# pycompression/python-zlib-ng

Measured on AMD Instinct MI355X. Metric: MB/s compress+decompress, 128 KiB blocks level 6, higher is better.
Workload: dtype u8

## Files before the change

### python-zlib-ng_amd/build.py

```python
import os
import subprocess
import sys

HERE = os.path.dirname(os.path.abspath(__file__))
CSRC = os.path.join(HERE, "csrc")
OUT = os.path.join(HERE, "zlib_ng_amd", "libzng_amd.so")
SOURCES = ["zng_amd.hip"]
DEPS = ["zng_amd.hip", "zng_stream.hip", "za_common.h", "za_crc.h", "za_deflate.hip", "za_inflate.hip", "za_inflate_units.hip", "za_inflate_spans.hip", "za_batch.hip", "za_dict.hip", "za_checksum.hip",
        os.path.join("..", "..", "include", "zng_amd.h")]


def needs_build():
    if not os.path.exists(OUT):
        return True
    t = os.path.getmtime(OUT)
    return any(os.path.getmtime(os.path.join(CSRC, d)) > t for d in DEPS)


def build(force=False, verbose=False):
    if not force and not needs_build():
        return OUT
    hipcc = os.environ.get("HIPCC", "/opt/rocm/bin/hipcc")
    cmd = [hipcc, "--offload-arch=gfx950", "-O3", "-std=c++17", "-fPIC", "-shared",
           "-Wall", "-Wno-unused-variable", "-Wno-unused-but-set-variable",
           "-o", OUT] + [os.path.join(CSRC, s) for s in SOURCES]
    if verbose:
        print(" ".join(cmd))
    subprocess.check_call(cmd)
    return OUT


def build_host_asan(out):
    hipcc = os.environ.get("HIPCC", "/opt/rocm/bin/hipcc")
    cmd = [hipcc, "--offload-arch=gfx950", "-Wno-option-ignored", "-O1", "-g", "-std=c++17", "-fPIC", "-shared", "-fsanitize=address,undefined",
           "-fno-sanitize-recover=undefined", "-fno-omit-frame-pointer", "-o", out] + [os.path.join(CSRC, s) for s in SOURCES]
    subprocess.check_call(cmd)
    return out


if __name__ == "__main__":
    if "--host-asan" in sys.argv:
        print(build_host_asan(sys.argv[sys.argv.index("--host-asan") + 1]))
    else:
        print(build(force="--force" in sys.argv, verbose=True))
```

### python-zlib-ng_amd/csrc/za_deflate.hip

```cpp
#include "za_common.h"
#include "za_crc.h"
#include <type_traits>

#define ZA_CH_GROUP 16
#define ZA_CH_OFFS(x) (((x) >> (32 - ZA_HASH_BITS - 2)) & (((1u << ZA_HASH_BITS) - 1u) << 2))
#define ZA_CH_CHUNK (64 * ZA_CH_GROUP)

typedef uint32_t za_v4u32 __attribute__((ext_vector_type(4)));
__device__ __forceinline__ void za_issue_load16(za_v4u32 &dst, const uint8_t *addr)
{
    asm volatile("global_load_dwordx4 %0, %1, off" : "=v"(dst) : "v"(addr) : "memory");
}
template <int NEWER>
__device__ __forceinline__ void za_wait_loads(za_v4u32 &a, za_v4u32 &b, za_v4u32 &c, za_v4u32 &d)
{
    asm volatile("s_waitcnt vmcnt(%4)" : "+v"(a), "+v"(b), "+v"(c), "+v"(d) : "n"(NEWER) : "memory");
}

__device__ __noinline__ uint32_t za_chains_fix(uint32_t h, uint32_t A, uint32_t old, bool ins)
{
    uint32_t near = 0, pre = 0xFFFFFFFFu;
    const int lane = za_lane();
    const unsigned long long insm = __ballot(ins);
    for (int j = 0; j < 64; j++) {
        const uint32_t hj = (uint32_t)__builtin_amdgcn_readlane((int)h, j), Aj = (uint32_t)__builtin_amdgcn_readlane((int)A, j);
        const uint32_t oj = (uint32_t)__builtin_amdgcn_readlane((int)old, j);
        if (((insm >> j) & 1ull) != 0ull && hj == h) {
            if (j < lane) near = Aj;
            pre = oj < pre ? oj : pre;
        }
    }
    return near ? near : pre;
}

#ifdef ZA_CH_STATS
__device__ unsigned long long za_ch_stat[32];
#endif
template <int TABLE>
__global__ __launch_bounds__(256) void za_k_chains(const uint8_t *__restrict__ in, const ZaUnit *__restrict__ units,
                                                   const uint32_t *__restrict__ run_start,
                                                   uint16_t *__restrict__ prev_ws,
                                                   uint32_t *__restrict__ cost_ws = nullptr)
{
    __shared__ uint32_t head[1 << ZA_HASH_BITS];
    __shared__ __attribute__((aligned(16))) uint32_t ring[(2 * ZA_CH_CHUNK + 16) / 4];
    __shared__ __attribute__((aligned(16))) uint16_t hbuf[2][ZA_CH_CHUNK];
    __shared__ __attribute__((aligned(16))) uint32_t obuf[2][ZA_CH_CHUNK];
    constexpr int HB = ZaTableBytes<TABLE>::value;
    const uint32_t lane = (uint32_t)za_lane();
    const uint32_t role = threadIdx.x >> 6;
    const uint32_t u0 = run_start[blockIdx.x], u1 = run_start[blockIdx.x + 1];
#ifdef ZA_CH_STATS
    unsigned long long st_wait = 0, st_ph[4] = {0, 0, 0, 0};
    const unsigned long long st_t0 = clock64();
#endif
    uint32_t goff = 0;
    uint32_t n_prev = 0;
#pragma unroll 1
    for (uint32_t ui = u0; ui < u1; ui++) {
        const ZaUnit u = units[ui];
        const int n = (int)u.in_len, dict_len = (int)u.dict_len;
        if (cost_ws && threadIdx.x == 0) cost_ws[(size_t)ui * ZA_DP_COSTS + 258] = 0u;
        const uint8_t *row = in + u.in_off - dict_len;
        uint16_t *prevdist = prev_ws + (size_t)ui * ZA_PREV_STRIDE;
#ifdef ZA_ABL_NO_CARRY
        const bool carry = false;
#else
        const bool carry = ui > u0 && (u.flags & ZA_FLAG_CARRY) != 0u;
#endif
        if (carry) goff += n_prev;
        else {
            goff = 0;
            for (uint32_t i = threadIdx.x * 4u; i < (1u << ZA_HASH_BITS); i += 1024u) *(uint4 *)&head[i] = make_uint4(0u, 0u, 0u, 0u);
        }
        __syncthreads();
        n_prev = (uint32_t)n;
        const int total = dict_len + n;
        const int first = carry ? dict_len - (HB - 1) : 0;
        const uint32_t abase = goff + (uint32_t)(2 * ZA_WIN - dict_len) + 1u;
        if (total < HB) {
            if (role == 2u && (int)lane >= first && (int)lane < total) prevdist[lane] = 0;
            continue;
        }
        if (total < 16) {
            if (role == 2u) {
                uint32_t h = 0xFFFFFFFFu;
                const bool ins = (int)lane >= first && (int)lane <= total - HB;
                if (ins) {
                    uint32_t w[3] = {0u, 0u, 0u};
#pragma unroll
                    for (int b = 0; b < HB; b++) w[b >> 2] |= (uint32_t)row[lane + b] << (8 * (b & 3));
                    h = za_hash_x<TABLE>(w[0], w[1], w[2]) >> (32 - ZA_HASH_BITS);
                }
                uint32_t d = 0;
                for (int j = 0; j < 16; j++) {
                    const uint32_t hj = (uint32_t)__builtin_amdgcn_readlane((int)h, j);
                    if (ins && j < (int)lane && hj == h) d = lane - (uint32_t)j;
                }
                if ((int)lane >= first && (int)lane < total) prevdist[lane] = (uint16_t)d;
            }
            continue;
        }
        const int iclamp_hi = total - HB;
        const int t0 = first & ~63;
        const int ngroups = (total - t0 + ZA_CH_CHUNK - 1) / ZA_CH_CHUNK;
        const int last16 = total - 16;
        auto fetch = [&](int c, za_v4u32 &dst) {
            int at = t0 + c * ZA_CH_CHUNK + 16 * (int)lane;
            at = at > last16 ? last16 : at;
            za_issue_load16(dst, row + at);
        };
        auto stage = [&](int c, uint4 v) {
            const int cbase = t0 + c * ZA_CH_CHUNK;
            if (cbase + ZA_CH_CHUNK > total) {
                const int at = cbase + 16 * (int)lane;
                const int delta = at > last16 ? at - last16 : 0;
                const uint32_t w[8] = {v.x, v.y, v.z, v.w, 0u, 0u, 0u, 0u};
                uint32_t r[4];
#pragma unroll
                for (int i = 0; i < 4; i++) {
                    uint32_t lo = 0, hi = 0;
#pragma unroll
                    for (int j = 0; j < 8; j++) { lo = (i + (delta >> 2)) == j ? w[j] : lo; hi = (i + (delta >> 2) + 1) == j ? w[j] : hi; }
                    r[i] = delta >= 16 ? 0u : __builtin_amdgcn_alignbyte(hi, lo, (uint32_t)delta & 3u);
                }
                v = make_uint4(r[0], r[1], r[2], r[3]);
            }
            *(uint4 *)(ring + (c & 1) * (ZA_CH_CHUNK / 4) + 4 * lane) = v;
            if ((c & 1) == 0 && lane == 0) *(uint4 *)(ring + 2 * ZA_CH_CHUNK / 4) = v;
        };
        auto hash_half = [&](int k, int g0, uint16_t *hb) {
#ifdef ZA_ABL_CH_NOHASH
            return;
#endif
            const uint32_t *w = ring + (k & 1) * (ZA_CH_CHUNK / 4) + 16 * g0 + lane;
            uint16_t *o = hb + 64 * g0 + 4 * lane;
#pragma unroll
            for (int j = 0; j < ZA_CH_GROUP / 8; j++) {
                const uint32_t d0 = w[64 * j], d1 = w[64 * j + 1];
                uint32_t hh[4];
                if constexpr (TABLE == ZA_TABLE_A) {
                    hh[0] = za_hash_x<TABLE>(d0, d1, 0u);
#pragma unroll
                    for (int q = 1; q < 4; q++) hh[q] = za_hash_x<TABLE>(__builtin_amdgcn_alignbyte(d1, d0, q), d1 >> (8 * q), 0u);
                } else if constexpr (TABLE == ZA_TABLE_B) {
                    hh[0] = za_hash_x<TABLE>(d0, 0u, 0u);
#pragma unroll
                    for (int q = 1; q < 4; q++) hh[q] = za_hash_x<TABLE>(__builtin_amdgcn_alignbyte(d1, d0, q), 0u, 0u);
                } else {
                    const uint32_t d2 = w[64 * j + 2], d3 = w[64 * j + 3];
                    hh[0] = za_hash_x<TABLE>(d0, d1, d2);
#pragma unroll
                    for (int q = 1; q < 4; q++)
                        hh[q] = za_hash_x<TABLE>(__builtin_amdgcn_alignbyte(d1, d0, q), __builtin_amdgcn_alignbyte(d2, d1, q), __builtin_amdgcn_alignbyte(d3, d2, q));
                }
                *(uint2 *)(o + 256 * j) = make_uint2(ZA_CH_OFFS(hh[0]) | (ZA_CH_OFFS(hh[1]) << 16), ZA_CH_OFFS(hh[2]) | (ZA_CH_OFFS(hh[3]) << 16));
            }
        };
        auto group_inner = [&](int k) -> bool {
            const int tbase = t0 + k * ZA_CH_CHUNK;
            return tbase >= first && tbase + ZA_CH_CHUNK - 1 <= iclamp_hi;
        };
        auto insert_as = [&](auto inner_tag, int tbase, const uint16_t *hb, uint32_t *ob) {
            constexpr bool inner = decltype(inner_tag)::value;
            const uint32_t li = (uint32_t)tbase + lane;
            uint32_t hh[ZA_CH_GROUP], old[ZA_CH_GROUP];
            const uint32_t A0 = abase + li;
#ifdef ZA_CH_STATS
            const unsigned long long T0 = clock64();
#endif
#ifdef ZA_ABL_CH_HALFREADS
#pragma unroll
            for (int g = 0; g < ZA_CH_GROUP; g += 2) { const uint32_t t = *(const uint32_t *)&hb[64 * g + 2 * (lane >> 1)]; hh[g] = t & 0xFFFCu; hh[g + 1] = (t >> 16) & 0xFFFCu; }
#else
#pragma unroll
            for (int g = 0; g < ZA_CH_GROUP; g++) hh[g] = hb[64 * g + lane];
#endif
#ifdef ZA_CH_STATS
            asm volatile("s_waitcnt lgkmcnt(0)" ::: "memory");
            const unsigned long long T1 = clock64();
#endif
#pragma unroll
            for (int g = 0; g < ZA_CH_GROUP; g++) {
                const int i = (int)li + 64 * g;
                const bool ins = inner || (i >= first && i <= iclamp_hi);
                old[g] = 0u;
#ifdef ZA_ABL_CH_NOATOMIC
                if (ins) old[g] = *(const uint32_t *)((const uint8_t *)head + hh[g]);
#else
                if (ins) old[g] = atomicMax((uint32_t *)((uint8_t *)head + hh[g]), A0 + 64u * (uint32_t)g);
#endif
            }
#ifdef ZA_CH_STATS
            asm volatile("s_waitcnt lgkmcnt(0)" ::: "memory");
            const unsigned long long T2 = clock64();
#endif
            uint32_t top = 0;
#pragma unroll
            for (int g = 0; g < ZA_CH_GROUP; g++) top |= (A0 + 64u * (uint32_t)g - old[g] - 1u);
#ifndef ZA_ABL_CH_NOCHECK
            if (__builtin_expect(__ballot((int)top < 0) != 0ull, 0)) {
#pragma unroll 1
                for (int g = 0; g < ZA_CH_GROUP; g++) {
                    const int i = (int)li + 64 * g;
                    const bool ins = inner || (i >= first && i <= iclamp_hi);
                    const uint32_t A = A0 + 64u * (uint32_t)g;
                    uint32_t hg = hh[0], og = old[0];
#pragma unroll
                    for (int q = 1; q < ZA_CH_GROUP; q++) { hg = g == q ? hh[q] : hg; og = g == q ? old[q] : og; }
                    const uint32_t ofix = za_chains_fix(hg >> 2, A, og, ins);
#pragma unroll
                    for (int q = 0; q < ZA_CH_GROUP; q++) old[q] = g == q ? ofix : old[q];
                }
            }
#endif
#ifdef ZA_ABL_CH_HALFWRITES
#pragma unroll
            for (int g = 0; g < ZA_CH_GROUP; g += 2) ob[64 * g + lane] = old[g] + old[g + 1];
#else
#pragma unroll
            for (int g = 0; g < ZA_CH_GROUP; g++) ob[64 * g + lane] = old[g];
#endif
#ifdef ZA_CH_STATS
            asm volatile("s_waitcnt lgkmcnt(0)" ::: "memory");
            st_ph[0] += T1 - T0; st_ph[1] += T2 - T1; st_ph[2] += clock64() - T2; st_ph[3] += 1;
#endif
        };
        auto store_links = [&](int k, uint32_t *ob) {
            const int tbase = t0 + k * ZA_CH_CHUNK;
            const uint32_t A0 = abase + (uint32_t)tbase + lane;
            uint32_t dd[ZA_CH_GROUP];
#pragma unroll
            for (int g = 0; g < ZA_CH_GROUP; g++) dd[g] = A0 + 64u * (uint32_t)g - ob[64 * g + lane];
            if (group_inner(k)) {
                uint16_t *lb = (uint16_t *)ob;
                __builtin_amdgcn_fence(__ATOMIC_ACQ_REL, "wavefront");
                __builtin_amdgcn_wave_barrier();
#pragma unroll
                for (int g = 0; g < ZA_CH_GROUP; g++) lb[64 * g + lane] = (uint16_t)(dd[g] <= (uint32_t)ZA_WIN ? dd[g] : 0u);
                __builtin_amdgcn_fence(__ATOMIC_ACQ_REL, "wavefront");
                __builtin_amdgcn_wave_barrier();
                const uint4 v0 = *(const uint4 *)&lb[8 * lane], v1 = *(const uint4 *)&lb[512 + 8 * lane];
#ifndef ZA_ABL_CH_NOSTORE
                *(uint4 *)(prevdist + tbase + 8 * (int)lane) = v0;
                *(uint4 *)(prevdist + tbase + 512 + 8 * (int)lane) = v1;
#endif
            } else {
#pragma unroll
                for (int g = 0; g < ZA_CH_GROUP; g++) {
                    const int i = tbase + (int)lane + 64 * g;
                    if (i >= first && i < total) prevdist[i] = (uint16_t)((i <= iclamp_hi && dd[g] <= (uint32_t)ZA_WIN) ? dd[g] : 0u);
                }
            }
        };
        auto wg_barrier = [&] {
#ifdef ZA_CH_STATS
            const unsigned long long b0 = clock64();
#endif
            __builtin_amdgcn_fence(__ATOMIC_RELEASE, "workgroup");
            __builtin_amdgcn_s_barrier();
            __builtin_amdgcn_fence(__ATOMIC_ACQUIRE, "workgroup");
#ifdef ZA_CH_STATS
            st_wait += clock64() - b0;
#endif
        };
        if (role == 0u) {
            za_v4u32 p0 = {0u, 0u, 0u, 0u}, p1 = p0, p2 = p0, p3 = p0;
            fetch(0, p0);
            za_wait_loads<0>(p0, p1, p2, p3);
            stage(0, make_uint4(p0.x, p0.y, p0.z, p0.w));
            fetch(1, p1); fetch(2, p2); fetch(3, p3); fetch(4, p0);
            wg_barrier();
            auto tick = [&](int t, za_v4u32 &pend) {
                if (t < ngroups) {
                    za_wait_loads<3>(p0, p1, p2, p3);
                    stage(t + 1, make_uint4(pend.x, pend.y, pend.z, pend.w));
                    fetch(t + 5, pend);
                    hash_half(t, ZA_CH_GROUP / 2, hbuf[t & 1]);
                }
                wg_barrier();
            };
#pragma unroll 1
            for (int t = 0; t <= ngroups + 1; t += 4) {
                tick(t, p1);
                if (t + 1 > ngroups + 1) break;
                tick(t + 1, p2);
                if (t + 2 > ngroups + 1) break;
                tick(t + 2, p3);
                if (t + 3 > ngroups + 1) break;
                tick(t + 3, p0);
            }
            za_wait_loads<0>(p0, p1, p2, p3);
        } else if (role == 1u) {
            wg_barrier();
#pragma unroll 1
            for (int t = 0; t <= ngroups + 1; t++) {
                if (t < ngroups) hash_half(t, 0, hbuf[t & 1]);
                wg_barrier();
            }
        } else if (role == 2u) {
            wg_barrier();
#pragma unroll 1
            for (int t = 0; t <= ngroups + 1; t++) {
                if (t >= 1 && t - 1 < ngroups) {
                    const int k = t - 1, tbase = t0 + k * ZA_CH_CHUNK;
                    if (group_inner(k)) insert_as(std::true_type{}, tbase, hbuf[k & 1], obuf[k & 1]);
                    else insert_as(std::false_type{}, tbase, hbuf[k & 1], obuf[k & 1]);
                }
                wg_barrier();
            }
        } else {
            wg_barrier();
#pragma unroll 1
            for (int t = 0; t <= ngroups + 1; t++) {
                if (t >= 2) store_links(t - 2, obuf[(t - 2) & 1]);
                wg_barrier();
            }
        }
    }
#ifdef ZA_CH_STATS
    if (lane == 0 && role == 2u && TABLE == 0) for (int i = 0; i < 4; i++) atomicAdd(&za_ch_stat[24 + i], st_ph[i]);
    if (lane == 0) { atomicAdd(&za_ch_stat[8 * TABLE + 2 * role], st_wait); atomicAdd(&za_ch_stat[8 * TABLE + 2 * role + 1], clock64() - st_t0); }
#endif
}

#ifndef ZA_SEARCH_CONSEC
#define ZA_SEARCH_CONSEC 1
#endif
#ifndef ZA_STATS_FOLD
#define ZA_STATS_FOLD 0
#endif
#define ZA_SEARCH_THREADS 1024
#define ZA_SEARCH_TILE    4096
#define ZA_RING           40960
#define ZA_BYTES          65536
#define ZA_LOOKAHEAD      272
#ifndef ZA_WL_STEPS
#define ZA_WL_STEPS       4
#endif
#define ZA_WL_ENTRIES     127
#define ZA_WL_BYTES       (16 * ZA_WL_ENTRIES * 8)

__device__ __forceinline__ uint32_t za_lds_ld32(const uint32_t *win32, uint32_t addr)
{
    const uint32_t idx = addr & (ZA_BYTES - 1), w = idx >> 2;
    return __builtin_amdgcn_alignbyte(win32[w + 1], win32[w], idx & 3u);
}


__device__ __forceinline__ int za_search_extend(const uint32_t *win32, uint32_t qb, uint32_t P, int len, int maxlen)
{
    {
        const uint32_t o = (uint32_t)len;
        const uint32_t is = (qb + o) & (ZA_BYTES - 1), ws = is >> 2, ip = (P + o) & (ZA_BYTES - 1), wp = ip >> 2;
        const uint32_t s0 = win32[ws], s1 = win32[ws + 1], s2 = win32[ws + 2], p0 = win32[wp], p1 = win32[wp + 1], p2 = win32[wp + 2];
        const uint32_t a0 = __builtin_amdgcn_alignbyte(s1, s0, is & 3u) ^ __builtin_amdgcn_alignbyte(p1, p0, ip & 3u);
        const uint32_t a1 = __builtin_amdgcn_alignbyte(s2, s1, is & 3u) ^ __builtin_amdgcn_alignbyte(p2, p1, ip & 3u);
        uint32_t g0, g1;
        asm("v_ffbl_b32 %0, %2\n\tv_ffbl_b32 %1, %3\n\tv_add_u32_e64 %1, %1, 32 clamp\n\tv_min_u32_e32 %0, %0, %1"
            : "=&v"(g0), "=&v"(g1) : "v"(a0), "v"(a1));
        const int nb = (int)min(g0 >> 3, 8u);
        len += nb;
        if (nb < 8 || len >= maxlen) return len < maxlen ? len : maxlen;
    }
    for (;;) {
        const uint32_t o = (uint32_t)len;
        const uint32_t is = (qb + o) & (ZA_BYTES - 1), ws = is >> 2, ip = (P + o) & (ZA_BYTES - 1), wp = ip >> 2;
        const uint32_t s0 = win32[ws], s1 = win32[ws + 1], s2 = win32[ws + 2], s3 = win32[ws + 3], s4 = win32[ws + 4];
        const uint32_t p0 = win32[wp], p1 = win32[wp + 1], p2 = win32[wp + 2], p3 = win32[wp + 3], p4 = win32[wp + 4];
        const uint32_t a0 = __builtin_amdgcn_alignbyte(s1, s0, is & 3u) ^ __builtin_amdgcn_alignbyte(p1, p0, ip & 3u);
        const uint32_t a1 = __builtin_amdgcn_alignbyte(s2, s1, is & 3u) ^ __builtin_amdgcn_alignbyte(p2, p1, ip & 3u);
        const uint32_t a2 = __builtin_amdgcn_alignbyte(s3, s2, is & 3u) ^ __builtin_amdgcn_alignbyte(p3, p2, ip & 3u);
        const uint32_t a3 = __builtin_amdgcn_alignbyte(s4, s3, is & 3u) ^ __builtin_amdgcn_alignbyte(p4, p3, ip & 3u);
        uint32_t g0, g1, g2, g3;
        asm("v_ffbl_b32 %0, %4\n\tv_ffbl_b32 %1, %5\n\tv_ffbl_b32 %2, %6\n\tv_ffbl_b32 %3, %7\n\t"
            "v_add_u32_e64 %1, %1, 32 clamp\n\tv_add_u32_e64 %2, %2, 64 clamp\n\tv_add_u32_e64 %3, %3, %8 clamp\n\t"
            "v_min3_u32 %0, %0, %1, %2\n\tv_min_u32_e32 %0, %0, %3"
            : "=&v"(g0), "=&v"(g1), "=&v"(g2), "=&v"(g3) : "v"(a0), "v"(a1), "v"(a2), "v"(a3), "s"(96u));
        const int nb = (int)min(g0 >> 3, 16u);
        len += nb;
        if (nb < 16 || len >= maxlen) break;
    }
    return len < maxlen ? len : maxlen;
}

__device__ __forceinline__ int za_ilog4(uint32_t a, uint32_t b)
{
    const uint32_t q = (a << 8) / b;
    const int lg = 23 - (int)__builtin_clz(q);
    const uint32_t t = q >> lg;
    return 4 * lg + (t >= 304u ? 1 : 0) + (t >= 362u ? 1 : 0) + (t >= 431u ? 1 : 0);
}

template <bool FULL, int STEPS = 0, bool USEC = false>
__global__ __launch_bounds__(ZA_SEARCH_THREADS) void za_k_search(const uint8_t *__restrict__ in, uint64_t in_total,
                                                                 const ZaUnit *__restrict__ units,
                                                                 const uint32_t *__restrict__ run_start,
                                                                 const uint16_t *__restrict__ prev_ws,
                                                                 const uint16_t *__restrict__ linkb_ws,
                                                                 const uint16_t *__restrict__ linkc_ws,
                                                                 uint32_t *__restrict__ best_ws, uint32_t *__restrict__ cost_ws, ZaLevel L)
{
    __shared__ __attribute__((aligned(16))) uint8_t lds[ZA_BYTES + 32 + 2 * ZA_RING + (FULL ? ZA_WL_BYTES : 0)];
    constexpr bool STATS = !FULL && ZA_STATS_FOLD;
    __shared__ uint32_t st_hist[STATS ? 256 : 1];
    __shared__ uint32_t st_cnt[4];
    uint32_t *win32 = (uint32_t *)lds;
    uint16_t *ring = (uint16_t *)(lds + ZA_BYTES + 32);
    constexpr uint32_t RING_B0 = ZA_BYTES + 32, RING_BYTES = 2 * ZA_RING;
    const int tid = (int)threadIdx.x;
    auto link_in = [](uint16_t v) -> uint16_t { return v ? v : (uint16_t)0xFFFFu; };
    auto quad_in = [](uint2 q) -> uint2 {
        uint2 r;
        asm("v_pk_sub_u16 %0, %2, %4\n\tv_pk_sub_u16 %1, %3, %4\n\tv_pk_add_u16 %0, %0, %4 clamp\n\tv_pk_add_u16 %1, %1, %4 clamp"
            : "=&v"(r.x), "=&v"(r.y) : "v"(q.x), "v"(q.y), "s"(0x00010001u));
        return r;
    };
    const uint32_t u0 = run_start[blockIdx.x], u1 = run_start[blockIdx.x + 1];
    uint32_t goff = 0;
    int carry_bytes = 0, n_prev = 0;
    const bool stats = STATS && L.dp != 0;
    if (stats) { if (tid < 256) st_hist[tid] = 0u; if (tid < 4) st_cnt[tid] = 0u; }
#pragma unroll 1
    for (uint32_t ui = u0; ui < u1; ui++) {
    const ZaUnit u = units[ui];
    const uint8_t *data = in + u.in_off;
    const int n = (int)u.in_len, dict_len = (int)u.dict_len;
    const uint16_t *prevdist = prev_ws + (size_t)ui * ZA_PREV_STRIDE;
    const uint16_t *linkb = linkb_ws + (size_t)ui * ZA_PREV_STRIDE + dict_len;
    const uint16_t *linkc = linkc_ws + (size_t)ui * ZA_PREV_STRIDE + dict_len;
    const int sshift = ZA_UNIT_SEG_SHIFT(u.flags);
    const bool carried = ui > u0;
    uint32_t *best = best_ws + (size_t)ui * ZA_BEST_STRIDE;
    const long long readable = (long long)(in_total - u.in_off);
    goff = carried ? goff + (uint32_t)n_prev : 0u;
    bool longm = false;
    int links_loaded = carried ? 0 : -dict_len;
    int bytes_loaded = carried ? carry_bytes - n_prev : (-dict_len) & ~3;
    if (carried && tid < ZA_HASH_BYTES_A - 1)
        ring[(goff + (uint32_t)(ZA_WIN - (ZA_HASH_BYTES_A - 1) + tid)) % ZA_RING] = link_in(prevdist[dict_len - (ZA_HASH_BYTES_A - 1) + tid]);
    auto load_quad = [&](int p, int limit) -> uint2 {
        uint2 q = make_uint2(0u, 0u);
        if (p < limit) { const ZaU2u t = *(const ZaU2u *)(prevdist + p + dict_len); q.x = t.x; q.y = t.y; }
        return q;
    };
    auto store_quad = [&](int p, int limit, uint2 q) {
        const uint32_t X = goff + (uint32_t)(ZA_WIN + p);
        q = quad_in(q);
        if ((X & 3u) == 0u && p + 4 <= limit) *(uint2 *)(lds + RING_B0 + 2u * (X % ZA_RING)) = q;
        else {
            for (int k = 0; k < 4; k++)
                if (p + k < limit) ring[(X + (uint32_t)k) % ZA_RING] = (uint16_t)((k < 2 ? q.x : q.y) >> (16 * (k & 1)));
        }
    };
    auto load_bytes = [&](int p) -> uint32_t {
        if (p >= -dict_len && (long long)p + 4 <= readable) return za_ld32(data + p);
        uint32_t v = 0;
        for (int k = 0; k < 4; k++)
            if (p + k >= -dict_len && (long long)(p + k) < readable) v |= (uint32_t)data[p + k] << (8 * k);
        return v;
    };
    auto store_bytes = [&](int p, uint32_t v) {
        const uint32_t w = ((goff + (uint32_t)(ZA_WIN + p)) & (ZA_BYTES - 1)) >> 2;
        win32[w] = v;
        if (w < 8) win32[w + ZA_BYTES / 4] = v;
    };
    {
        int need_links = ZA_SEARCH_TILE < n ? ZA_SEARCH_TILE : n;
        for (int p = links_loaded + 4 * tid; p < need_links; p += 4 * ZA_SEARCH_THREADS) store_quad(p, need_links, load_quad(p, need_links));
        links_loaded = need_links;
        int need_bytes = ZA_SEARCH_TILE + ZA_LOOKAHEAD;
        if (need_bytes > n) need_bytes = n;
        need_bytes = (need_bytes + 3) & ~3;
        if ((carried || bytes_loaded == -dict_len) && (long long)need_bytes <= readable)
            for (int p = bytes_loaded + 4 * tid; p < need_bytes; p += 4 * ZA_SEARCH_THREADS) store_bytes(p, za_ld32(data + p));
        else
            for (int p = bytes_loaded + 4 * tid; p < need_bytes; p += 4 * ZA_SEARCH_THREADS) store_bytes(p, load_bytes(p));
        bytes_loaded = need_bytes;
    }
#ifndef ZA_OWN_STAGE
#define ZA_OWN_STAGE 0
#endif
    za_v4u32 oq = {0u, 0u, 0u, 0u};
    auto own_area = [&](int tile_base) -> uint32_t { return (goff + (uint32_t)(ZA_WIN + tile_base) + 4608u + 15u) & 0xFFF0u; };
    auto own_load = [&](int tile_base) {
        const bool forc = tid >= ZA_SEARCH_THREADS / 2;
        const int p = tile_base + 8 * (tid & (ZA_SEARCH_THREADS / 2 - 1));
        oq = za_v4u32{0u, 0u, 0u, 0u};
#ifdef ZA_ABL_NO_LINKLOADS
        oq.x = oq.y = oq.z = oq.w = (((uint32_t)p * 7u & 0xFFu) | 1u) * 0x00010001u;
#else
        if (p < n && (USEC || !forc)) { const ZaU4u t = *(const ZaU4u *)((forc ? linkc : linkb) + p); oq.x = t.x; oq.y = t.y; oq.z = t.z; oq.w = t.w; }
#endif
    };
    auto own_store = [&](int tile_base) {
        const uint32_t a = (own_area(tile_base) + (tid >= ZA_SEARCH_THREADS / 2 ? 8192u : 0u) + 16u * (uint32_t)(tid & (ZA_SEARCH_THREADS / 2 - 1))) & 0xFFFFu;
        *(uint4 *)(lds + a) = make_uint4(oq.x, oq.y, oq.z, oq.w);
    };
    uint32_t nlkb[ZA_SEARCH_TILE / ZA_SEARCH_THREADS], nlkc[ZA_SEARCH_TILE / ZA_SEARCH_THREADS];
    constexpr bool CONSEC = !FULL && ZA_SEARCH_CONSEC && !ZA_OWN_STAGE && !ZA_STATS_FOLD;
    uint2 nob = make_uint2(0u, 0u), noc = make_uint2(0u, 0u);
    auto load_own_links = [&](int tile_base) {
        if (ZA_OWN_STAGE) { own_load(tile_base); return; }
        if (CONSEC) {
            const int p = tile_base + 4 * tid;
            const uint32_t off = 2u * (uint32_t)(p < n ? p : (n - 1) & ~3);
#ifdef ZA_ABL_NO_LINKLOADS
            nob = make_uint2(0x00010001u, 0x00010001u); noc = nob;
#else
            if (n > 0) { const ZaU2u t = *(const ZaU2u *)((const uint8_t *)linkb + off); nob.x = t.x; nob.y = t.y; }
            if (USEC && n > 0) { const ZaU2u t = *(const ZaU2u *)((const uint8_t *)linkc + off); noc.x = t.x; noc.y = t.y; }
#endif
            return;
        }
#pragma unroll
        for (int k = 0; k < ZA_SEARCH_TILE / ZA_SEARCH_THREADS; k++) {
            const int p = tile_base + k * ZA_SEARCH_THREADS + tid;
#ifdef ZA_ABL_NO_LINKLOADS
            nlkb[k] = ((uint32_t)p * 7u & 0xFFu) | 1u; nlkc[k] = ((uint32_t)p * 13u & 0x3FFu) | 1u;
#else
            const uint32_t off = 2u * (uint32_t)(p < n ? p : n - 1);
            nlkb[k] = n > 0 ? (uint32_t)*(const uint16_t *)((const uint8_t *)linkb + off) : 0u;
            nlkc[k] = USEC && n > 0 ? (uint32_t)*(const uint16_t *)((const uint8_t *)linkc + off) : 0u;
#endif
        }
    };
    load_own_links(0);
    if (ZA_OWN_STAGE) own_store(0);
    uint32_t res[ZA_SEARCH_TILE / ZA_SEARCH_THREADS];
    int res_base = -1;
    auto flush_results = [&]() {
        if (res_base < 0) return;
        if (CONSEC) {
            const int p = res_base + 4 * tid;
            if (p + 4 <= n) *(uint4 *)(best + p) = make_uint4(res[0], res[1], res[2], res[3]);
            else {
#pragma unroll
                for (int k = 0; k < 4; k++) if (p + k < n) best[p + k] = res[k];
            }
            res_base = -1;
            return;
        }
#pragma unroll
        for (int k = 0; k < ZA_SEARCH_TILE / ZA_SEARCH_THREADS; k++) {
            const int p = res_base + k * ZA_SEARCH_THREADS + tid;
            if (p < n) best[p] = res[k];
        }
        res_base = -1;
    };
    uint32_t st_e = 0u, st_pe = 0u, st_U = 0u, st_NM = 0u;
    bool st_have = false;
    auto stats_issue = [&](int tile_base) {
        const int p = tile_base + ((tid >> 8) << 10) + (tid & 255);
        st_have = p < n;
        st_e = 0u; st_pe = 0u;
        if (st_have) { st_e = best[p]; if (p > 0) st_pe = best[p - 1]; }
    };
    auto stats_use = [&]() {
        const uint32_t len = ZA_ELEN(st_e), lp = ZA_ELEN(st_pe);
        if (st_have) {
            if (len == 0u || (len == 3u && ZA_EDIST(st_e) > (uint32_t)ZA_DP_WEAK_DIST)) { atomicAdd(&st_hist[st_e >> 24], 1u); st_U++; }
            else if (len + 1u != lp) st_NM++;
        }
        st_have = false;
    };
    __syncthreads();
    for (int base = 0; base < n; base += ZA_SEARCH_TILE) {
        uint32_t lkb[ZA_SEARCH_TILE / ZA_SEARCH_THREADS], lkc[ZA_SEARCH_TILE / ZA_SEARCH_THREADS];
#pragma unroll
        for (int k = 0; k < ZA_SEARCH_TILE / ZA_SEARCH_THREADS; k++) {
            if (ZA_OWN_STAGE) {
                const uint32_t a = own_area(base) + 2u * (uint32_t)(k * ZA_SEARCH_THREADS + tid);
                lkb[k] = *(const uint16_t *)(lds + (a & 0xFFFFu));
                lkc[k] = USEC ? (uint32_t)*(const uint16_t *)(lds + ((a + 8192u) & 0xFFFFu)) : 0u;
            } else if (CONSEC) {
                lkb[k] = ((k < 2 ? nob.x : nob.y) >> (16 * (k & 1))) & 0xFFFFu;
                lkc[k] = ((k < 2 ? noc.x : noc.y) >> (16 * (k & 1))) & 0xFFFFu;
            } else { lkb[k] = nlkb[k]; lkc[k] = nlkc[k]; }
            asm volatile("" : "+v"(lkb[k]), "+v"(lkc[k]) : : "memory");
        }
        if (ZA_OWN_STAGE) za_lds_barrier();
        if constexpr (!FULL) flush_results();
        int need_links = base + 2 * ZA_SEARCH_TILE;
        if (need_links > n) need_links = n;
        int need_bytes = base + 2 * ZA_SEARCH_TILE + ZA_LOOKAHEAD;
        if (need_bytes > n) need_bytes = n;
        need_bytes = (need_bytes + 3) & ~3;
        uint64_t nbv; uint32_t nsh;
        const int pq = links_loaded + 4 * tid;
        const uint2 nq = load_quad(pq, need_links);
        {
            const int rd_i = (int)(readable < (long long)0x7FFFFFF0 ? readable : (long long)0x7FFFFFF0);
            const int p = bytes_loaded + 8 * tid;
            int over = p + 8 - rd_i;
            over = over > 0 ? over : 0;
            nbv = 0ull; nsh = 8u * (uint32_t)over;
            if (p < need_bytes) nbv = za_ld64(data + p - over);
        }
        if constexpr (FULL) {
        const int lane = tid & 63;
        uint32_t *wl = (uint32_t *)(lds + ZA_BYTES + 32 + 2 * ZA_RING) + (tid >> 6) * (2 * ZA_WL_ENTRIES);
        uint32_t wl_n = 0;
        auto visit = [&](uint32_t P, uint32_t me0, uint32_t me1, uint32_t me2, uint32_t me3, int maxlen, int cap, int nice,
                         uint32_t &q, uint32_t &qb, uint32_t &d, int &best_len, int &best_dist, int &depth) -> bool {
            bool alive = depth > 0;
            int steps = ZA_WL_STEPS;
#pragma unroll
            while (alive && steps-- > 0) {
                depth--;
                q -= d;
                qb -= 2u * d;
                qb += qb < RING_B0 ? RING_BYTES : 0u;
                const int dist = (int)(P - q);
                if (dist > L.max_dist) { alive = false; break; }
                d = *(const uint16_t *)(lds + qb);
                const uint32_t sh = q & 3u;
                const uint32_t *cw = (const uint32_t *)(lds + (q & (uint32_t)(ZA_BYTES - 4)));
                const uint32_t c0 = cw[0], c1 = cw[1], c2 = cw[2], c3 = cw[3], c4 = cw[4];
// ... 1740 lines not shown
```

Before: 56480.

## Rebalance hash-chain pipeline roles and swizzle LDS layouts for wide accesses

Moves the hash-chain overflow fix-up out of the insert stage into the link-building stage, which now works on halves and recomputes hashes from the row when needed. The hashing work is spread over three wave roles instead of two, and both link halves are split across two roles. LDS hash and old-position buffers use XOR-swizzled row layouts so insert and link stages can read and write with 16-byte vector accesses and fewer bank conflicts. This balances per-stage work across the four-wave pipeline, at the cost of more intricate indexing and a fix-up path that recomputes hashes.

```diff
diff --git a/python-zlib-ng_amd/build.py b/python-zlib-ng_amd/build.py
--- a/python-zlib-ng_amd/build.py
+++ b/python-zlib-ng_amd/build.py
@@ -17,13 +17,17 @@
     return any(os.path.getmtime(os.path.join(CSRC, d)) > t for d in DEPS)
 
 
+def command(out=OUT, defines=()):
+    hipcc = os.environ.get("HIPCC", "/opt/rocm/bin/hipcc")
+    return [hipcc, "--offload-arch=gfx950", "-O3", "-std=c++17", "-fPIC", "-shared",
+            "-Wall", "-Wno-unused-variable", "-Wno-unused-but-set-variable"] + list(defines) + \
+           ["-o", out] + [os.path.join(CSRC, s) for s in SOURCES]
+
+
 def build(force=False, verbose=False):
     if not force and not needs_build():
         return OUT
-    hipcc = os.environ.get("HIPCC", "/opt/rocm/bin/hipcc")
-    cmd = [hipcc, "--offload-arch=gfx950", "-O3", "-std=c++17", "-fPIC", "-shared",
-           "-Wall", "-Wno-unused-variable", "-Wno-unused-but-set-variable",
-           "-o", OUT] + [os.path.join(CSRC, s) for s in SOURCES]
+    cmd = command()
     if verbose:
         print(" ".join(cmd))
     subprocess.check_call(cmd)
diff --git a/python-zlib-ng_amd/csrc/za_deflate.hip b/python-zlib-ng_amd/csrc/za_deflate.hip
--- a/python-zlib-ng_amd/csrc/za_deflate.hip
+++ b/python-zlib-ng_amd/csrc/za_deflate.hip
@@ -5,6 +5,8 @@
 #define ZA_CH_GROUP 16
 #define ZA_CH_OFFS(x) (((x) >> (32 - ZA_HASH_BITS - 2)) & (((1u << ZA_HASH_BITS) - 1u) << 2))
 #define ZA_CH_CHUNK (64 * ZA_CH_GROUP)
+#define ZA_CH_HROW(l, p) (16u * ((l) ^ (((l) >> 2) & 3u)) + 8u * (((p) ^ ((l) >> 3) ^ ((l) >> 5)) & 1u))
+#define ZA_CH_OROW(l, p) (16u * (l) + 4u * (((p) ^ ((l) >> 1) ^ (((l) >> 3) & 1u)) & 3u))
 
 typedef uint32_t za_v4u32 __attribute__((ext_vector_type(4)));
 __device__ __forceinline__ void za_issue_load16(za_v4u32 &dst, const uint8_t *addr)
@@ -108,7 +110,9 @@
         auto fetch = [&](int c, za_v4u32 &dst) {
             int at = t0 + c * ZA_CH_CHUNK + 16 * (int)lane;
             at = at > last16 ? last16 : at;
+#ifndef ZA_ABL_CH_NOLOAD
             za_issue_load16(dst, row + at);
+#endif
         };
         auto stage = [&](int c, uint4 v) {
             const int cbase = t0 + c * ZA_CH_CHUNK;
@@ -129,14 +133,18 @@
             *(uint4 *)(ring + (c & 1) * (ZA_CH_CHUNK / 4) + 4 * lane) = v;
             if ((c & 1) == 0 && lane == 0) *(uint4 *)(ring + 2 * ZA_CH_CHUNK / 4) = v;
         };
-        auto hash_half = [&](int k, int g0, uint16_t *hb) {
+        auto hash_part = [&](auto nq_tag, int k, int g0, uint16_t *hb) {
 #ifdef ZA_ABL_CH_NOHASH
             return;
 #endif
+            constexpr int NQ = decltype(nq_tag)::value;
             const uint32_t *w = ring + (k & 1) * (ZA_CH_CHUNK / 4) + 16 * g0 + lane;
-            uint16_t *o = hb + 64 * g0 + 4 * lane;
-#pragma unroll
-            for (int j = 0; j < ZA_CH_GROUP / 8; j++) {
+            const uint32_t i = lane & 15u, piece = (uint32_t)(g0 >> 3);
+            uint16_t *o = hb + (g0 & 7) + (lane >> 4);
+            uint16_t *const o0 = o + ZA_CH_HROW(4u * i + 0u, piece), *const o1 = o + ZA_CH_HROW(4u * i + 1u, piece);
+            uint16_t *const o2 = o + ZA_CH_HROW(4u * i + 2u, piece), *const o3 = o + ZA_CH_HROW(4u * i + 3u, piece);
+#pragma unroll
+            for (int j = 0; j < NQ; j++) {
                 const uint32_t d0 = w[64 * j], d1 = w[64 * j + 1];
                 uint32_t hh[4];
                 if constexpr (TABLE == ZA_TABLE_A) {
@@ -154,7 +162,8 @@
                     for (int q = 1; q < 4; q++)
                         hh[q] = za_hash_x<TABLE>(__builtin_amdgcn_alignbyte(d1, d0, q), __builtin_amdgcn_alignbyte(d2, d1, q), __builtin_amdgcn_alignbyte(d3, d2, q));
                 }
-                *(uint2 *)(o + 256 * j) = make_uint2(ZA_CH_OFFS(hh[0]) | (ZA_CH_OFFS(hh[1]) << 16), ZA_CH_OFFS(hh[2]) | (ZA_CH_OFFS(hh[3]) << 16));
+                o0[4 * j] = (uint16_t)ZA_CH_OFFS(hh[0]); o1[4 * j] = (uint16_t)ZA_CH_OFFS(hh[1]);
+                o2[4 * j] = (uint16_t)ZA_CH_OFFS(hh[2]); o3[4 * j] = (uint16_t)ZA_CH_OFFS(hh[3]);
             }
         };
         auto group_inner = [&](int k) -> bool {
@@ -162,6 +171,9 @@
             return tbase >= first && tbase + ZA_CH_CHUNK - 1 <= iclamp_hi;
         };
         auto insert_as = [&](auto inner_tag, int tbase, const uint16_t *hb, uint32_t *ob) {
+#ifdef ZA_ABL_CH_NOINSERT
+            return;
+#endif
             constexpr bool inner = decltype(inner_tag)::value;
             const uint32_t li = (uint32_t)tbase + lane;
             uint32_t hh[ZA_CH_GROUP], old[ZA_CH_GROUP];
@@ -169,13 +181,17 @@
 #ifdef ZA_CH_STATS
             const unsigned long long T0 = clock64();
 #endif
-#ifdef ZA_ABL_CH_HALFREADS
-#pragma unroll
-            for (int g = 0; g < ZA_CH_GROUP; g += 2) { const uint32_t t = *(const uint32_t *)&hb[64 * g + 2 * (lane >> 1)]; hh[g] = t & 0xFFFCu; hh[g + 1] = (t >> 16) & 0xFFFCu; }
+            {
+                const uint4 a = *(const uint4 *)(hb + ZA_CH_HROW(lane, 0u)), b = *(const uint4 *)(hb + ZA_CH_HROW(lane, 1u));
+                const uint32_t w[8] = {a.x, a.y, a.z, a.w, b.x, b.y, b.z, b.w};
+#ifdef ZA_ABL_CH_NOHASH
+                constexpr uint32_t m = 0xFFFCu;
 #else
-#pragma unroll
-            for (int g = 0; g < ZA_CH_GROUP; g++) hh[g] = hb[64 * g + lane];
-#endif
+                constexpr uint32_t m = 0xFFFFu;
+#endif
+#pragma unroll
+                for (int g = 0; g < ZA_CH_GROUP; g += 2) { hh[g] = w[g >> 1] & m; hh[g + 1] = (w[g >> 1] >> 16) & m; }
+            }
 #ifdef ZA_CH_STATS
             asm volatile("s_waitcnt lgkmcnt(0)" ::: "memory");
             const unsigned long long T1 = clock64();
@@ -195,60 +211,78 @@
             asm volatile("s_waitcnt lgkmcnt(0)" ::: "memory");
             const unsigned long long T2 = clock64();
 #endif
-            uint32_t top = 0;
-#pragma unroll
-            for (int g = 0; g < ZA_CH_GROUP; g++) top |= (A0 + 64u * (uint32_t)g - old[g] - 1u);
-#ifndef ZA_ABL_CH_NOCHECK
-            if (__builtin_expect(__ballot((int)top < 0) != 0ull, 0)) {
-#pragma unroll 1
-                for (int g = 0; g < ZA_CH_GROUP; g++) {
-                    const int i = (int)li + 64 * g;
-                    const bool ins = inner || (i >= first && i <= iclamp_hi);
-                    const uint32_t A = A0 + 64u * (uint32_t)g;
-                    uint32_t hg = hh[0], og = old[0];
-#pragma unroll
-                    for (int q = 1; q < ZA_CH_GROUP; q++) { hg = g == q ? hh[q] : hg; og = g == q ? old[q] : og; }
-                    const uint32_t ofix = za_chains_fix(hg >> 2, A, og, ins);
-#pragma unroll
-                    for (int q = 0; q < ZA_CH_GROUP; q++) old[q] = g == q ? ofix : old[q];
-                }
-            }
-#endif
-#ifdef ZA_ABL_CH_HALFWRITES
-#pragma unroll
-            for (int g = 0; g < ZA_CH_GROUP; g += 2) ob[64 * g + lane] = old[g] + old[g + 1];
-#else
-#pragma unroll
-            for (int g = 0; g < ZA_CH_GROUP; g++) ob[64 * g + lane] = old[g];
-#endif
+#pragma unroll
+            for (int p = 0; p < ZA_CH_GROUP / 4; p++)
+                *(uint4 *)(ob + ZA_CH_OROW(lane, (uint32_t)p)) = make_uint4(old[4 * p], old[4 * p + 1], old[4 * p + 2], old[4 * p + 3]);
 #ifdef ZA_CH_STATS
             asm volatile("s_waitcnt lgkmcnt(0)" ::: "memory");
             st_ph[0] += T1 - T0; st_ph[1] += T2 - T1; st_ph[2] += clock64() - T2; st_ph[3] += 1;
 #endif
         };
-        auto store_links = [&](int k, uint32_t *ob) {
-            const int tbase = t0 + k * ZA_CH_CHUNK;
-            const uint32_t A0 = abase + (uint32_t)tbase + lane;
-            uint32_t dd[ZA_CH_GROUP];
-#pragma unroll
-            for (int g = 0; g < ZA_CH_GROUP; g++) dd[g] = A0 + 64u * (uint32_t)g - ob[64 * g + lane];
-            if (group_inner(k)) {
-                uint16_t *lb = (uint16_t *)ob;
+        auto make_links = [&](auto half_tag, int k, uint32_t *ob) {
+#ifdef ZA_ABL_CH_NOLINKS
+            return;
+#endif
+            constexpr int H = decltype(half_tag)::value, NG = ZA_CH_GROUP / 2;
+            const int tbase = t0 + k * ZA_CH_CHUNK, hbase = tbase + 64 * NG * H;
+            const bool inner = group_inner(k);
+            const uint32_t li = (uint32_t)hbase + lane;
+            const uint32_t A0 = abase + li;
+            uint32_t old[NG];
+            {
+                const uint4 a = *(const uint4 *)(ob + ZA_CH_OROW(lane, 2u * H)), b = *(const uint4 *)(ob + ZA_CH_OROW(lane, 2u * H + 1u));
+                old[0] = a.x; old[1] = a.y; old[2] = a.z; old[3] = a.w; old[4] = b.x; old[5] = b.y; old[6] = b.z; old[7] = b.w;
+            }
+            uint32_t top = 0;
+#pragma unroll
+            for (int g = 0; g < NG; g++) top |= (A0 + 64u * (uint32_t)g - old[g] - 1u);
+#ifdef ZA_CH_FORCE_FIX
+            const bool fix = true;
+#elif defined(ZA_ABL_CH_NOCHECK)
+            const bool fix = false;
+#else
+            const bool fix = __builtin_expect(__ballot((int)top < 0) != 0ull, 0);
+#endif
+            if (fix) {
+#pragma unroll 1
+                for (int g = 0; g < NG; g++) {
+                    const int i = (int)li + 64 * g;
+                    const bool ins = inner || (i >= first && i <= iclamp_hi);
+                    uint32_t h = 0xFFFFFFFFu;
+                    if (ins) {
+                        uint32_t w[3] = {0u, 0u, 0u};
+#pragma unroll
+                        for (int b = 0; b < HB; b++) w[b >> 2] |= (uint32_t)row[i + b] << (8 * (b & 3));
+                        h = za_hash_x<TABLE>(w[0], w[1], w[2]) >> (32 - ZA_HASH_BITS);
+                    }
+                    uint32_t og = old[0];
+#pragma unroll
+                    for (int q = 1; q < NG; q++) og = g == q ? old[q] : og;
+                    const uint32_t ofix = za_chains_fix(h, A0 + 64u * (uint32_t)g, og, ins);
+#pragma unroll
+                    for (int q = 0; q < NG; q++) old[q] = g == q ? (ins ? ofix : 0u) : old[q];
+                }
+            }
+            uint32_t dd[NG];
+#pragma unroll
+            for (int g = 0; g < NG; g++) dd[g] = A0 + 64u * (uint32_t)g - old[g];
+            if (inner) {
+                uint16_t *lb = (uint16_t *)ob + (lane & 7u);
+                uint16_t *const lb0 = lb + 2u * ZA_CH_OROW(lane >> 3, 2u * H), *const lb1 = lb + 2u * ZA_CH_OROW(8u + (lane >> 3), 2u * H);
                 __builtin_amdgcn_fence(__ATOMIC_ACQ_REL, "wavefront");
                 __builtin_amdgcn_wave_barrier();
 #pragma unroll
-                for (int g = 0; g < ZA_CH_GROUP; g++) lb[64 * g + lane] = (uint16_t)(dd[g] <= (uint32_t)ZA_WIN ? dd[g] : 0u);
+                for (int g = 0; g < NG; g++) ((g & 1) ? lb1 : lb0)[512 * (g >> 1)] = (uint16_t)(dd[g] <= (uint32_t)ZA_WIN ? dd[g] : 0u);
                 __builtin_amdgcn_fence(__ATOMIC_ACQ_REL, "wavefront");
                 __builtin_amdgcn_wave_barrier();
-                const uint4 v0 = *(const uint4 *)&lb[8 * lane], v1 = *(const uint4 *)&lb[512 + 8 * lane];
+                const uint4 v = *(const uint4 *)(ob + ZA_CH_OROW(lane, 2u * H));
 #ifndef ZA_ABL_CH_NOSTORE
-                *(uint4 *)(prevdist + tbase + 8 * (int)lane) = v0;
-                *(uint4 *)(prevdist + tbase + 512 + 8 * (int)lane) = v1;
+                *(uint4 *)(prevdist + hbase + 8 * (int)lane) = v;
 #endif
             } else {
 #pragma unroll
-                for (int g = 0; g < ZA_CH_GROUP; g++) {
-                    const int i = tbase + (int)lane + 64 * g;
+                for (int g = 0; g < NG; g++) {
+                    const int i = (int)li + 64 * g;
                     if (i >= first && i < total) prevdist[i] = (uint16_t)((i <= iclamp_hi && dd[g] <= (uint32_t)ZA_WIN) ? dd[g] : 0u);
                 }
             }
@@ -276,7 +310,7 @@
                     za_wait_loads<3>(p0, p1, p2, p3);
                     stage(t + 1, make_uint4(pend.x, pend.y, pend.z, pend.w));
                     fetch(t + 5, pend);
-                    hash_half(t, ZA_CH_GROUP / 2, hbuf[t & 1]);
+                    hash_part(std::integral_constant<int, 2>{}, t, ZA_CH_GROUP / 2, hbuf[t & 1]);
                 }
                 wg_barrier();
             };
@@ -295,7 +329,8 @@
             wg_barrier();
 #pragma unroll 1
             for (int t = 0; t <= ngroups + 1; t++) {
-                if (t < ngroups) hash_half(t, 0, hbuf[t & 1]);
+                if (t < ngroups) hash_part(std::integral_constant<int, 1>{}, t, 0, hbuf[t & 1]);
+                if (t >= 2) make_links(std::integral_constant<int, 1>{}, t - 2, obuf[(t - 2) & 1]);
                 wg_barrier();
             }
         } else if (role == 2u) {
@@ -313,7 +348,8 @@
             wg_barrier();
 #pragma unroll 1
             for (int t = 0; t <= ngroups + 1; t++) {
-                if (t >= 2) store_links(t - 2, obuf[(t - 2) & 1]);
+                if (t < ngroups) hash_part(std::integral_constant<int, 1>{}, t, ZA_CH_GROUP / 4, hbuf[t & 1]);
+                if (t >= 2) make_links(std::integral_constant<int, 0>{}, t - 2, obuf[(t - 2) & 1]);
                 wg_barrier();
             }
         }
```

New measurement: 56500, median of 3. Within noise of the previous version (+0.0%).
